# lmcinnes/pynndescent

Hardware: AMD Instinct MI355X
Metric: index build: points indexed/sec (recall@10 vs brute force reported alongside) (higher is better)
Workload: dtype f32

## Files before the change

pynndescent_amd/csrc/sample.hip:

```cpp
#include "common.h"
#include "state.h"

__device__ __forceinline__ uint32_t nnd_offer_salt(uint32_t it_seed, uint32_t u) { return nnd_hash2(it_seed ^ 0x3C6EF372u, u); }

__device__ __forceinline__ uint32_t nnd_offer_slot(uint32_t salt_u, uint32_t v, int rcap) { return nnd_hash2(salt_u ^ 0x68E31DA4u, v) & (uint32_t)(rcap - 1); }
__device__ __forceinline__ int64_t nnd_offer_addr(uint32_t u, uint32_t cls, uint32_t salt_u, uint32_t v, int rcap, int wide) {
    return wide ? (int64_t)u * 2 * rcap + nnd_offer_slot(salt_u, v, 2 * rcap) : ((int64_t)u * 2 + cls) * rcap + nnd_offer_slot(salt_u, v, rcap);
}
__device__ __forceinline__ uint64_t nnd_offer_key(uint32_t slot_word, uint32_t salt_u) {
    return ((uint64_t)slot_word << 32) | (uint64_t)(nnd_unmix32(slot_word) ^ salt_u);
}

__global__ __launch_bounds__(256) void k_sample_reverse(const uint32_t *__restrict__ knn_e, int64_t row_lo, int64_t n, int k, int ks, uint32_t it_seed,
                                                        uint32_t *__restrict__ rbuf, int rcap, int64_t own_lo, int64_t own_hi, int pass,
                                                        uint8_t *__restrict__ active, const int32_t *__restrict__ order, int wide) {
    int64_t b = blockIdx.x;
    if ((gridDim.x & 7) == 0) b = (b & 7) * (gridDim.x >> 3) + (b >> 3);
    const int64_t g = row_lo + b * blockDim.y + threadIdx.y;
    const int j = threadIdx.x;
    if (g >= n || j >= k) return;
    const int64_t v = order ? (int64_t)order[g] : g;
    uint32_t e = knn_e[v * ks + j];
    if (e == NND_EMPTY_E) return;
    uint32_t u = e & NND_IDX_MASK;
    uint32_t cls = e >> 31;
    if (cls != (uint32_t)(pass == 0)) return;
    if (pass == 0 && v >= own_lo && v < own_hi) active[v] = 1;
    if ((int64_t)u < own_lo || (int64_t)u >= own_hi) return;
    if (pass == 0) active[u] = 1;
    else if (!active[u]) return;
    const uint32_t salt = nnd_offer_salt(it_seed, u);
    atomicMin(&rbuf[nnd_offer_addr(u, cls, salt, (uint32_t)v, rcap, wide)], nnd_mix32((uint32_t)v ^ salt));
}

#define SAMPLE_MAX_ITEMS 128

struct sample_scratch {
    uint64_t key[2][SAMPLE_MAX_ITEMS];
};

__global__ __launch_bounds__(256) void k_sample_select(uint32_t *__restrict__ knn_e, int64_t n, int k, int ks, int mc,
                                                       int mcp, uint32_t it_seed, uint32_t *__restrict__ rbuf, int rcap,
                                                       int32_t *__restrict__ cand, int64_t own_lo, int64_t own_hi,
                                                       const uint8_t *__restrict__ active, int wide) {
    __shared__ sample_scratch scr[4];
    const int lane = nnd_lane(), w = threadIdx.x >> 6;
    const int64_t v = own_lo + (int64_t)blockIdx.x * 4 + w;
    if (v >= own_hi) return;
    sample_scratch &sc = scr[w];
    if (!active[v]) {
        for (int j = lane; j < mcp; j += 64) cand[v * 2 * mcp + j] = -1;
        return;
    }

    uint32_t e = NND_EMPTY_E;
    if (lane < k) e = knn_e[v * ks + lane];
    const bool valid = e != NND_EMPTY_E;
    const uint32_t u = e & NND_IDX_MASK;
    const uint32_t cls = e >> 31;
    const uint64_t fkey = ((uint64_t)nnd_hash3(it_seed, (uint32_t)v, u) << 32) | u;
    int cnt[2];
#pragma unroll
    for (int c = 0; c < 2; c++) {
        bool mine = valid && cls == (uint32_t)c;
        unsigned long long m = __ballot(mine);
        if (mine) sc.key[c][nnd_prefix_popc(m)] = fkey;
        cnt[c] = __popcll(m);
    }
    nnd_wave_lds_sync();
    const int nfwd[2] = {cnt[0], cnt[1]};
    const uint32_t salt = nnd_offer_salt(it_seed, (uint32_t)v);
    if (2 * rcap <= 64) {
        const int c = (wide || lane >= rcap) ? 1 : 0;
        uint32_t *slots = rbuf + v * 2 * rcap;
        uint32_t rw = NND_EMPTY_SLOT;
        if (lane < 2 * rcap) {
            rw = slots[lane];
            if (rw != NND_EMPTY_SLOT) slots[lane] = NND_EMPTY_SLOT;
        }
        bool ok = rw != NND_EMPTY_SLOT;
        const uint64_t rk = nnd_offer_key(rw, salt);
        if (ok) {
            const uint32_t src = (uint32_t)rk;
            const int nf = c ? nfwd[1] : nfwd[0];
            for (int j = 0; j < nf; j++) ok &= ((uint32_t)sc.key[c][j] != src);
        }
#pragma unroll
        for (int cc = 0; cc < 2; cc++) {
            const bool mine = ok && c == cc;
            const unsigned long long m = __ballot(mine);
            if (mine) sc.key[cc][cnt[cc] + nnd_prefix_popc(m)] = rk;
            cnt[cc] += __popcll(m);
        }
    } else {
#pragma unroll
        for (int c = 0; c < 2; c++) {
            uint32_t *slots = rbuf + (v * 2 + c) * rcap;
            for (int s0 = 0; s0 < rcap; s0 += 64) {
                int s = s0 + lane;
                uint32_t rw = NND_EMPTY_SLOT;
                if (s < rcap) {
                    rw = slots[s];
                    if (rw != NND_EMPTY_SLOT) slots[s] = NND_EMPTY_SLOT;
                }
                bool ok = rw != NND_EMPTY_SLOT;
                const uint64_t rk = nnd_offer_key(rw, salt);
                if (ok) {
                    uint32_t src = (uint32_t)rk;
                    for (int j = 0; j < nfwd[c]; j++) ok &= ((uint32_t)sc.key[c][j] != src);
                }
                unsigned long long m = __ballot(ok);
                if (ok) sc.key[c][cnt[c] + nnd_prefix_popc(m)] = rk;
                cnt[c] += __popcll(m);
            }
        }
    }
    nnd_wave_lds_sync();

    int32_t *out = cand + v * 2 * mcp;
    int my_rank = 1 << 30;
    const int my_item = (valid && cls == 1u) ? nnd_prefix_popc(__ballot(valid && cls == 1u)) : -1;
#pragma unroll
    for (int c = 0; c < 2; c++) {
        const int M = cnt[c];
        int32_t *dst = out + (c == 1 ? 0 : mcp);
        for (int i0 = 0; i0 < M; i0 += 64) {
            int i = i0 + lane;
            int r = 1 << 30;
            uint64_t key = 0;
            if (i < M) {
                key = sc.key[c][i];
                r = 0;
                for (int j = 0; j < M; j++) r += (sc.key[c][j] < key) ? 1 : 0;
                if (r < mc) dst[r] = (int32_t)(uint32_t)key;
            }
            if (c == 1 && i0 == 0) {
                const int got = __shfl(r, my_item >= 0 ? my_item : 0, 64);
                if (my_item >= 0) my_rank = got;
            }
        }
        int filled = M < mc ? M : mc;
        for (int j = filled + lane; j < mcp; j += 64) dst[j] = -1;
    }
    if (valid && cls == 1u && my_rank < mc) knn_e[v * ks + lane] = u;
}

__global__ __launch_bounds__(256) void k_sample_select_wide(uint32_t *__restrict__ knn_e, int64_t n, int k, int ks, int mc,
                                                            int mcp, uint32_t it_seed, uint32_t *__restrict__ rbuf, int rcap,
                                                            int32_t *__restrict__ cand, int64_t own_lo, int64_t own_hi,
                                                            const uint8_t *__restrict__ active) {
    constexpr int MAXI = NND_WIDE_K + 128;
    __shared__ uint64_t skey[4][2][MAXI];
    __shared__ int srank[4][NND_WIDE_K];
    const int lane = nnd_lane(), w = threadIdx.x >> 6;
    const int64_t v = own_lo + (int64_t)blockIdx.x * 4 + w;
    if (v >= own_hi) return;
    if (!active[v]) {
        for (int j = lane; j < mcp; j += 64) cand[v * 2 * mcp + j] = -1;
        return;
    }
    uint64_t(*key)[MAXI] = skey[w];
    uint32_t e[NND_WIDE_U];
    int item[NND_WIDE_U];
    int cnt[2] = {0, 0};
#pragma unroll
    for (int u = 0; u < NND_WIDE_U; u++) {
        const int j = lane + 64 * u;
        e[u] = j < k ? knn_e[v * ks + j] : NND_EMPTY_E;
        item[u] = -1;
    }
#pragma unroll
    for (int c = 0; c < 2; c++) {
#pragma unroll
        for (int u = 0; u < NND_WIDE_U; u++) {
            const bool mine = e[u] != NND_EMPTY_E && (e[u] >> 31) == (uint32_t)c;
            const unsigned long long m = __ballot(mine);
            if (mine) {
                const uint32_t tgt = e[u] & NND_IDX_MASK;
                item[u] = cnt[c] + nnd_prefix_popc(m);
                key[c][item[u]] = ((uint64_t)nnd_hash3(it_seed, (uint32_t)v, tgt) << 32) | tgt;
            }
            cnt[c] += __popcll(m);
        }
    }
    nnd_wave_lds_sync();
    const int nfwd[2] = {cnt[0], cnt[1]};
    const uint32_t salt = nnd_offer_salt(it_seed, (uint32_t)v);
#pragma unroll
    for (int c = 0; c < 2; c++) {
        uint32_t *slots = rbuf + (v * 2 + c) * rcap;
        for (int s0 = 0; s0 < rcap; s0 += 64) {
            const int sidx = s0 + lane;
            uint32_t rw = NND_EMPTY_SLOT;
            if (sidx < rcap) {
                rw = slots[sidx];
                if (rw != NND_EMPTY_SLOT) slots[sidx] = NND_EMPTY_SLOT;
            }
            bool ok = rw != NND_EMPTY_SLOT;
            const uint64_t rk = nnd_offer_key(rw, salt);
            if (__ballot(ok)) {
                const uint32_t src = (uint32_t)rk;
                for (int j = 0; j < nfwd[c]; j++) ok = ok && ((uint32_t)key[c][j] != src);
            }
            const unsigned long long m = __ballot(ok);
            if (ok) key[c][cnt[c] + nnd_prefix_popc(m)] = rk;
            cnt[c] += __popcll(m);
        }
    }
    nnd_wave_lds_sync();
    int32_t *out = cand + v * 2 * mcp;
#pragma unroll
    for (int c = 0; c < 2; c++) {
        const int M = cnt[c];
        int32_t *dst = out + (c == 1 ? 0 : mcp);
        for (int i0 = 0; i0 < M; i0 += 64) {
            const int i = i0 + lane;
            if (i < M) {
                const uint64_t kk = key[c][i];
                int r = 0;
                for (int j = 0; j < M; j++) r += (key[c][j] < kk) ? 1 : 0;
                if (r < mc) dst[r] = (int32_t)(uint32_t)kk;
                if (c == 1 && i < nfwd[1]) srank[w][i] = r;
            }
        }
        const int filled = M < mc ? M : mc;
        for (int j = filled + lane; j < mcp; j += 64) dst[j] = -1;
    }
    nnd_wave_lds_sync();
#pragma unroll
    for (int u = 0; u < NND_WIDE_U; u++) {
        const int j = lane + 64 * u;
        if (e[u] != NND_EMPTY_E && (e[u] >> 31) == 1u && item[u] >= 0 && srank[w][item[u]] < mc) knn_e[v * ks + j] = e[u] & NND_IDX_MASK;
    }
}

template <bool WIDE>
__device__ __forceinline__ void nnd_select_half(uint32_t *__restrict__ knn_e, int k, int ks, int mc, int mcp, uint32_t it_seed,
                                                int32_t *__restrict__ cand, int64_t vv, bool act, uint32_t e, uint32_t rw0, uint32_t rw1,
                                                uint64_t (*sk)[64], int j, int hb) {
    const uint32_t salt = nnd_offer_salt(it_seed, (uint32_t)vv);
    const uint64_t rk0 = nnd_offer_key(rw0, salt), rk1 = nnd_offer_key(rw1, salt);
    const bool valid = e != NND_EMPTY_E;
    const uint32_t u = e & NND_IDX_MASK;
    const uint32_t cls = e >> 31;
    const uint64_t fkey = ((uint64_t)nnd_hash3(it_seed, (uint32_t)vv, u) << 32) | u;
    const uint32_t below = (1u << j) - 1u;
    int cnt[2];
    uint32_t fmask1 = 0;
#pragma unroll
    for (int c = 0; c < 2; c++) {
        const bool mine = valid && cls == (uint32_t)c;
        const uint32_t hm = (uint32_t)(__ballot(mine) >> hb);
        if (mine) sk[c][__popc(hm & below)] = fkey;
        cnt[c] = __popc(hm);
        if (c == 1) fmask1 = hm;
    }
    nnd_wave_lds_sync();
    const int nf0 = cnt[0], nf1 = cnt[1];
    int32_t *out = cand + vv * 2 * mcp;
    int my_rank = 1 << 30;
    const int my_item = (valid && cls == 1u) ? __popc(fmask1 & below) : -1;
    if constexpr (WIDE) {
        uint64_t *fl = &sk[0][0];
        const uint64_t fk = j < nf1 ? sk[1][j] : NND_EMPTY_KEY;
        nnd_wave_lds_sync();
        if (j < nf1) fl[j] = fk;
        nnd_wave_lds_sync();
        bool ok0 = rw0 != NND_EMPTY_SLOT, ok1 = rw1 != NND_EMPTY_SLOT;
        {
            const int a0 = __builtin_amdgcn_readlane(nf1, 0), a1 = __builtin_amdgcn_readlane(nf1, 32);
            const int nfm = a0 > a1 ? a0 : a1;
            const uint32_t s0 = (uint32_t)rk0, s1 = (uint32_t)rk1;
            for (int q = 0; q < nfm; q++) {
                const uint32_t f = (uint32_t)fl[q];
                ok0 = ok0 && !(q < nf1 && f == s0);
                ok1 = ok1 && !(q < nf1 && f == s1);
            }
        }
        int M = nf1;
        {
            const uint32_t hm0 = (uint32_t)(__ballot(ok0) >> hb), hm1 = (uint32_t)(__ballot(ok1) >> hb);
            if (ok0) fl[M + __popc(hm0 & below)] = rk0;
            M += __popc(hm0);
            if (ok1) fl[M + __popc(hm1 & below)] = rk1;
            M += __popc(hm1);
        }
        nnd_wave_lds_sync();
        const int m0 = __builtin_amdgcn_readlane(M, 0), m1 = __builtin_amdgcn_readlane(M, 32);
        const int mm = m0 > m1 ? m0 : m1;
        const uint64_t key0 = j < M ? fl[j] : NND_EMPTY_KEY, key1 = 32 + j < M ? fl[32 + j] : NND_EMPTY_KEY, key2 = 64 + j < M ? fl[64 + j] : NND_EMPTY_KEY;
        int r0 = 0, r1 = 0, r2 = 0;
        for (int q = 0; q < mm; q++) {
            const uint64_t kq = fl[q];
            const bool in = q < M;
            r0 += (in && kq < key0) ? 1 : 0;
            r1 += (in && kq < key1) ? 1 : 0;
            r2 += (in && kq < key2) ? 1 : 0;
        }
        if (act) {
            if (j < M && r0 < mc) out[r0] = (int32_t)(uint32_t)key0;
            if (32 + j < M && r1 < mc) out[r1] = (int32_t)(uint32_t)key1;
            if (64 + j < M && r2 < mc) out[r2] = (int32_t)(uint32_t)key2;
            const int filled = M < mc ? M : mc;
            for (int q = filled + j; q < mcp; q += 32) out[q] = -1;
            for (int q = j; q < mcp; q += 32) out[mcp + q] = -1;
        }
        const int got = __builtin_amdgcn_ds_bpermute((hb + (my_item >= 0 ? my_item : 0)) << 2, r0);
        if (my_item >= 0) my_rank = got;
        if (act && valid && cls == 1u && my_rank < mc) knn_e[vv * ks + j] = u;
        return;
    }
    bool ok0 = rw0 != NND_EMPTY_SLOT, ok1 = rw1 != NND_EMPTY_SLOT;
    {
        const int a = nf0 > nf1 ? nf0 : nf1;
        const int a0 = __builtin_amdgcn_readlane(a, 0), a1 = __builtin_amdgcn_readlane(a, 32);
        const int nfm = a0 > a1 ? a0 : a1;
        const uint32_t s0 = (uint32_t)rk0, s1 = (uint32_t)rk1;
        for (int q = 0; q < nfm; q++) {
            const uint32_t f0 = (uint32_t)sk[0][q], f1 = (uint32_t)sk[1][q];
            ok0 = ok0 && !(q < nf0 && f0 == s0);
            ok1 = ok1 && !(q < nf1 && f1 == s1);
        }
    }
    {
        const uint32_t hm0 = (uint32_t)(__ballot(ok0) >> hb), hm1 = (uint32_t)(__ballot(ok1) >> hb);
        if (ok0) sk[0][cnt[0] + __popc(hm0 & below)] = rk0;
        if (ok1) sk[1][cnt[1] + __popc(hm1 & below)] = rk1;
        cnt[0] += __popc(hm0);
        cnt[1] += __popc(hm1);
    }
    nnd_wave_lds_sync();

#pragma unroll
    for (int c = 0; c < 2; c++) {
        const int M = cnt[c];
        const int m0 = __builtin_amdgcn_readlane(M, 0), m1 = __builtin_amdgcn_readlane(M, 32);
        const int mm = m0 > m1 ? m0 : m1;
        int32_t *dst = out + (c == 1 ? 0 : mcp);
        const uint64_t key0 = j < M ? sk[c][j] : NND_EMPTY_KEY, key1 = 32 + j < M ? sk[c][32 + j] : NND_EMPTY_KEY;
        int r0 = 0, r1 = 0;
        for (int q = 0; q < mm; q++) {
            const uint64_t kq = sk[c][q];
            const bool in = q < M;
            r0 += (in && kq < key0) ? 1 : 0;
            r1 += (in && kq < key1) ? 1 : 0;
        }
        if (act) {
            if (j < M && r0 < mc) dst[r0] = (int32_t)(uint32_t)key0;
            if (32 + j < M && r1 < mc) dst[r1] = (int32_t)(uint32_t)key1;
            const int filled = M < mc ? M : mc;
            for (int q = filled + j; q < mcp; q += 32) dst[q] = -1;
        }
        if (c == 1) {
            const int got = __builtin_amdgcn_ds_bpermute((hb + (my_item >= 0 ? my_item : 0)) << 2, r0);
            if (my_item >= 0) my_rank = got;
        }
    }
    if (act && valid && cls == 1u && my_rank < mc) knn_e[vv * ks + j] = u;
}

template <int LW>
__device__ __forceinline__ int nnd_group_max(int v) {
    int m = __builtin_amdgcn_readlane(v, 0);
#pragma unroll
    for (int g = LW; g < 64; g += LW) {
        const int o = __builtin_amdgcn_readlane(v, g);
        m = o > m ? o : m;
    }
    return m;
}
template <int LW, int NR>
__device__ __forceinline__ int nnd_select_class(bool act, bool fvalid, uint64_t fkey, const bool (&rvalid)[NR], const uint64_t (&rkey)[NR], int mc,
                                                int mcp, int32_t *dst, uint64_t *list, int j, int gb) {
    constexpr uint32_t GM = LW == 32 ? 0xFFFFFFFFu : ((1u << (LW & 31)) - 1u);
    constexpr int CAP = 2 * LW;
    uint64_t *F = list, *C = list + LW;
    const uint32_t below = (1u << j) - 1u;
    const uint32_t fmask = (uint32_t)(__ballot(fvalid) >> gb) & GM;
    const int nf = __popc(fmask);
    if (fvalid) F[__popc(fmask & below)] = fkey;
    int M = nf;
#pragma unroll
    for (int i = 0; i < NR; i++) M += __popc((uint32_t)(__ballot(rvalid[i]) >> gb) & GM);
    const uint32_t fp = (uint32_t)(fkey >> 32);
    uint32_t rp[NR];
#pragma unroll
    for (int i = 0; i < NR; i++) rp[i] = (uint32_t)(rkey[i] >> 32);
    uint32_t tau = 0xFFFFFFFFu, lo = 0u, hi = 0xFFFFFFFFu;
    if (M > CAP || M > 2 * mc + 4) {
        const float t = (float)(mc + 10) * 4294967296.0f / (float)M;
        tau = t >= 4294967040.0f ? 0xFFFFFFFFu : (uint32_t)t;
    }
    const int nfm = nnd_group_max<LW>(nf);
    int count = 0, cv = 0, tpos = -1, cn = 0;
    uint64_t key0 = NND_EMPTY_KEY, key1 = NND_EMPTY_KEY;
    bool dup0 = false, dup1 = false;
#pragma unroll 1
    for (int iter = 0; iter < 30; iter++) {
        nnd_wave_lds_sync();
        const bool fpass = fvalid && fp <= tau;
        const uint32_t pm = (uint32_t)(__ballot(fpass) >> gb) & GM;
        const int npf = __popc(pm);
        tpos = fpass ? __popc(pm & below) : -1;
        if (fpass) C[tpos] = fkey;
        int pos = npf;
#pragma unroll
        for (int i = 0; i < NR; i++) {
            const bool rpass = rvalid[i] && rp[i] <= tau;
            const uint32_t m = (uint32_t)(__ballot(rpass) >> gb) & GM;
            const int p = pos + __popc(m & below);
            if (rpass && p < CAP) C[p] = rkey[i];
            pos += __popc(m);
        }
        count = pos;
        nnd_wave_lds_sync();
        cn = count < CAP ? count : CAP;
        const bool two = nnd_group_max<LW>(cn) > LW;
        key0 = j < cn ? C[j] : NND_EMPTY_KEY;
        key1 = (two && LW + j < cn) ? C[LW + j] : NND_EMPTY_KEY;
        const bool rev0 = j >= npf && j < cn, rev1 = two && LW + j < cn;
        dup0 = dup1 = false;
        if (__ballot(rev0 || rev1)) {
            const uint32_t s0 = (uint32_t)key0, s1 = (uint32_t)key1;
            if (two) {
#pragma unroll 4
                for (int q = 0; q < nfm; q++) {
                    const uint32_t f = (uint32_t)F[q];
                    dup0 = dup0 || (rev0 && q < nf && f == s0);
                    dup1 = dup1 || (rev1 && q < nf && f == s1);
                }
            } else {
#pragma unroll 4
                for (int q = 0; q < nfm; q++) dup0 = dup0 || (rev0 && q < nf && (uint32_t)F[q] == s0);
            }
        }
        cv = cn - __popc((uint32_t)(__ballot(dup0) >> gb) & GM) - __popc((uint32_t)(__ballot(dup1) >> gb) & GM);
        const bool ok = count <= CAP && (cv >= mc || tau == 0xFFFFFFFFu);
        if (!__ballot(!ok)) break;
        if (!ok) {
            if (count > CAP) {
                hi = tau;
                tau = lo + (hi - lo) / 2;
            } else {
                lo = tau;
                const uint64_t up = (uint64_t)tau + (tau >> 1) + 1u;
                tau = hi == 0xFFFFFFFFu ? (up >= 0xFFFFFFFFull ? 0xFFFFFFFFu : (uint32_t)up) : lo + (hi - lo) / 2 + 1u;
            }
        }
    }
    if (dup0) key0 = NND_EMPTY_KEY;
    if (dup1) key1 = NND_EMPTY_KEY;
    const int cmax = nnd_group_max<LW>(cn);
    nnd_wave_lds_sync();
    C[j] = key0;
    if (cmax > LW) C[LW + j] = key1;
    nnd_wave_lds_sync();
    int r0 = 0, r1 = 0;
    if (cmax > LW) {
#pragma unroll 4
        for (int q = 0; q < cmax; q++) {
            const uint64_t kq = C[q];
            const bool in = q < cn;
            r0 += (in && kq < key0) ? 1 : 0;
            r1 += (in && kq < key1) ? 1 : 0;
        }
    } else {
#pragma unroll 4
        for (int q = 0; q < cmax; q++) r0 += (q < cn && C[q] < key0) ? 1 : 0;
    }
    if (act) {
        if (key0 != NND_EMPTY_KEY && r0 < mc) dst[r0] = (int32_t)(uint32_t)key0;
        if (key1 != NND_EMPTY_KEY && r1 < mc) dst[r1] = (int32_t)(uint32_t)key1;
        const int filled = cv < mc ? cv : mc;
        for (int q = filled + j; q < mcp; q += LW) dst[q] = -1;
    }
    const int got = __builtin_amdgcn_ds_bpermute((gb + (tpos >= 0 ? tpos : 0)) << 2, r0);
    return tpos >= 0 ? got : (1 << 30);
}

template <bool WIDE, int LW, int NRC>
__device__ __forceinline__ void nnd_select_group(uint32_t *__restrict__ knn_e, int k, int ks, int mc, int mcp, uint32_t it_seed,
                                                 int32_t *__restrict__ cand, int64_t vv, bool act, uint32_t e, const uint32_t (&rwo)[NRC],
                                                 const uint32_t (&rwn)[NRC], uint64_t *list, int j, int gb) {
    const uint32_t salt = nnd_offer_salt(it_seed, (uint32_t)vv);
    const bool valid = e != NND_EMPTY_E;
    const uint32_t u = e & NND_IDX_MASK;
    const uint32_t cls = e >> 31;
    const uint64_t fkey = ((uint64_t)nnd_hash3(it_seed, (uint32_t)vv, u) << 32) | u;
    int32_t *out = cand + vv * 2 * mcp;
    int my_rank;
    if constexpr (WIDE) {
        bool rv[2 * NRC];
        uint64_t rk[2 * NRC];
#pragma unroll
        for (int i = 0; i < NRC; i++) {
            rv[i] = rwo[i] != NND_EMPTY_SLOT;
            rk[i] = nnd_offer_key(rwo[i], salt);
            rv[NRC + i] = rwn[i] != NND_EMPTY_SLOT;
            rk[NRC + i] = nnd_offer_key(rwn[i], salt);
        }
        my_rank = nnd_select_class<LW, 2 * NRC>(act, valid, fkey, rv, rk, mc, mcp, out, list, j, gb);
        if (act)
            for (int q = j; q < mcp; q += LW) out[mcp + q] = -1;
    } else {
        bool rv0[NRC], rv1[NRC];
        uint64_t rk0[NRC], rk1[NRC];
#pragma unroll
        for (int i = 0; i < NRC; i++) {
            rv0[i] = rwo[i] != NND_EMPTY_SLOT;
            rk0[i] = nnd_offer_key(rwo[i], salt);
            rv1[i] = rwn[i] != NND_EMPTY_SLOT;
            rk1[i] = nnd_offer_key(rwn[i], salt);
        }
        (void)nnd_select_class<LW, NRC>(act, valid && cls == 0u, fkey, rv0, rk0, mc, mcp, out + mcp, list, j, gb);
        my_rank = nnd_select_class<LW, NRC>(act, valid && cls == 1u, fkey, rv1, rk1, mc, mcp, out, list, j, gb);
    }
    if (act && valid && cls == 1u && my_rank < mc) knn_e[vv * ks + j] = u;
}

template <bool WIDE>
__global__ __launch_bounds__(256) void k_sample_select_h(uint32_t *__restrict__ knn_e, int64_t n, int k, int ks, int mc,
                                                         int mcp, uint32_t it_seed, uint32_t *__restrict__ rbuf,
                                                         int32_t *__restrict__ cand, int64_t own_lo, int64_t own_hi,
                                                         const uint8_t *__restrict__ active) {
    constexpr int RCAP = 32;
    __shared__ uint64_t skey[8][2][64];
    const int lane = nnd_lane(), w = threadIdx.x >> 6, h = lane >> 5, j = lane & 31, hb = lane & 32;
    const int64_t v = own_lo + ((int64_t)blockIdx.x * 4 + w) * 2 + h;
    const bool von = v < own_hi;
    const bool act = von && active[von ? v : own_lo] != 0;
    if (von && !act)
        for (int q = j; q < mcp; q += 32) cand[v * 2 * mcp + q] = -1;
    if (!__ballot(act)) return;
    uint64_t(*sk)[64] = skey[w * 2 + h];
    const int64_t vv = act ? v : own_lo;

    uint32_t e = NND_EMPTY_E;
    if (act && j < k) e = knn_e[vv * ks + j];
    uint32_t rw0 = NND_EMPTY_SLOT, rw1 = NND_EMPTY_SLOT;
    uint32_t *slots = rbuf + vv * 2 * RCAP;
    if (act) {
        rw0 = slots[j];
        rw1 = slots[RCAP + j];
        if (rw0 != NND_EMPTY_SLOT) slots[j] = NND_EMPTY_SLOT;
        if (rw1 != NND_EMPTY_SLOT) slots[RCAP + j] = NND_EMPTY_SLOT;
    }
    nnd_select_half<WIDE>(knn_e, k, ks, mc, mcp, it_seed, cand, vv, act, e, rw0, rw1, sk, j, hb);
}

#define RV_TAB 1024
#ifndef RV_RPT
#define RV_RPT 8
#endif
#define RV_NOHASH 0xFFFFu
#ifndef RV_SEL_THREADS
#define RV_SEL_THREADS 512
#endif

__device__ __forceinline__ uint32_t rv_tab_hash(uint32_t b) { return (b * 2654435761u) >> 22; }

__device__ __forceinline__ int rv_tab_find(volatile uint32_t *hkey, uint32_t b) {
    uint32_t h = rv_tab_hash(b);
#pragma unroll 1
    for (int p = 0; p < 24; p++) {
        uint32_t cur = hkey[h];
        if (cur == 0xFFFFFFFFu) cur = atomicCAS((uint32_t *)&hkey[h], 0xFFFFFFFFu, b);
        if (cur == 0xFFFFFFFFu || cur == b) return (int)h;
        h = (h + 1) & (RV_TAB - 1);
    }
    return -1;
}
#define RV_NOKEY 0xFFFFFFFFu
__device__ __forceinline__ void rv_row_groups(uint32_t key, int &rank, int &size, int &leader) {
    const int lane = (int)__builtin_amdgcn_mbcnt_hi(~0u, __builtin_amdgcn_mbcnt_lo(~0u, 0u));
    rank = 0;
    size = 1;
    leader = lane;
#define RV_ROT(r)                                                                         \
    {                                                                                     \
        const uint32_t ok = (uint32_t)nnd_dpp_i32<NND_DPP_ROW_ROR(r)>((int)key);           \
        const int ol = nnd_dpp_i32<NND_DPP_ROW_ROR(r)>(lane);                              \
        const bool eq = ok == key;                                                        \
        size += eq ? 1 : 0;                                                               \
        rank += (eq && ol < lane) ? 1 : 0;                                                \
        leader = (eq && ol < leader) ? ol : leader;                                       \
    }
    RV_ROT(1) RV_ROT(2) RV_ROT(3) RV_ROT(4) RV_ROT(5) RV_ROT(6) RV_ROT(7) RV_ROT(8)
    RV_ROT(9) RV_ROT(10) RV_ROT(11) RV_ROT(12) RV_ROT(13) RV_ROT(14) RV_ROT(15)
#undef RV_ROT
}
__device__ __forceinline__ uint32_t rv_offer_word(uint32_t it_seed, uint32_t u, uint32_t v) { return nnd_mix32(v ^ nnd_offer_salt(it_seed, u)); }

__global__ __launch_bounds__(256) void k_rev_mark(const uint32_t *__restrict__ knn_e, int64_t row0, int64_t n_rows, int ks, uint8_t *__restrict__ active) {
    const int64_t i = ((int64_t)blockIdx.x * 256 + threadIdx.x) * 4;
    if (i >= n_rows * ks) return;
    const u32x4 e = *(const u32x4 *)(knn_e + row0 * ks + i);
    const int64_t v = row0 + i / ks;
#pragma unroll
    for (int q = 0; q < 4; q++) {
        const uint32_t w = e[q];
        if (w != NND_EMPTY_E && (w >> 31)) {
            active[v] = 1;
            const uint32_t t = w & NND_IDX_MASK;
            if ((uint32_t)(t - (uint32_t)row0) < (uint32_t)n_rows) active[t] = 1;
        }
    }
}
__global__ void k_rev_mark_records(const int32_t *__restrict__ targets, int64_t count, int64_t row0, int64_t n_rows, uint8_t *__restrict__ active) {
    const int64_t i = (int64_t)blockIdx.x * blockDim.x + threadIdx.x;
    if (i >= count) return;
    const uint32_t t = (uint32_t)targets[i];
    const uint32_t u = t & NND_IDX_MASK;
    if ((t >> 31) && (uint32_t)(u - (uint32_t)row0) < (uint32_t)n_rows) active[u] = 1;
}

struct rv_inbox {
    const uint32_t *cursor = nullptr;
    const uint2 *rec = nullptr;
    int cap = 0;
    const uint2 *ov = nullptr;
    const uint32_t *ov_count = nullptr;
};
__global__ __launch_bounds__(256) void k_rev_place(const uint32_t *__restrict__ knn_e, int64_t row0, int64_t n, int k, int ks, uint32_t it_seed,
                                                   const int32_t *__restrict__ order, const int32_t *__restrict__ pos, int logB,
                                                   uint8_t *__restrict__ active, int mark, uint32_t *__restrict__ in_cursor,
                                                   uint2 *__restrict__ in_rec, int cap, uint2 *__restrict__ ov, uint32_t *__restrict__ ov_count) {
    __shared__ uint32_t hkey[RV_TAB], hcnt[RV_TAB], hbase[RV_TAB];
    const int tid = threadIdx.y * blockDim.x + threadIdx.x;
    for (int i = tid; i < RV_TAB; i += 256) { hkey[i] = 0xFFFFFFFFu; hcnt[i] = 0; }
    __syncthreads();
    const int j = threadIdx.x;
    const uint32_t sub = blockIdx.x & 7u, bmask = (1u << logB) - 1u;
    uint32_t ev[RV_RPT], vv[RV_RPT];
#pragma unroll
    for (int it = 0; it < RV_RPT; it++) {
        const int64_t g = ((int64_t)blockIdx.x * RV_RPT + it) * blockDim.y + threadIdx.y;
        ev[it] = NND_EMPTY_E;
        vv[it] = 0;
        if (g < n && j < k) {
            vv[it] = (uint32_t)(order ? order[g] : (int32_t)(row0 + g));
            ev[it] = knn_e[(int64_t)vv[it] * ks + j];
        }
    }
    uint32_t bb[RV_RPT], w[RV_RPT], at[RV_RPT];
    uint16_t m[RV_RPT], hh[RV_RPT];
#pragma unroll
    for (int it = 0; it < RV_RPT; it++) {
        bb[it] = RV_NOKEY;
        w[it] = at[it] = 0;
        m[it] = 0;
        hh[it] = RV_NOHASH;
        if (ev[it] != NND_EMPTY_E && (uint32_t)((ev[it] & NND_IDX_MASK) - (uint32_t)row0) >= (uint32_t)n) {
            if ((ev[it] >> 31) && mark == 1) active[vv[it]] = 1;
            ev[it] = NND_EMPTY_E;
        }
        if (ev[it] != NND_EMPTY_E) {
            const uint32_t u = ev[it] & NND_IDX_MASK, cls = ev[it] >> 31;
            if (cls && mark == 1) { active[vv[it]] = 1; active[u] = 1; }
            if (mark == 2 && !cls && !active[u]) ev[it] = NND_EMPTY_E;
        }
        if (ev[it] != NND_EMPTY_E) {
            const uint32_t u = ev[it] & NND_IDX_MASK, cls = ev[it] >> 31;
            const uint32_t ul = u - (uint32_t)row0;
            const uint32_t p = (uint32_t)(pos ? pos[ul] : (int32_t)ul);
            bb[it] = p >> logB;
            w[it] = rv_offer_word(it_seed, u, vv[it]);
            m[it] = (uint16_t)((p & bmask) | (cls << 15));
        }
    }
#pragma unroll
    for (int it = 0; it < RV_RPT; it++) {
        int rank, size, leader;
        rv_row_groups(bb[it], rank, size, leader);
        int h = -1;
        uint32_t base = 0;
        if (bb[it] != RV_NOKEY && rank == 0) {
            h = rv_tab_find(hkey, bb[it]);
            base = h >= 0 ? atomicAdd(&hcnt[h], (uint32_t)size) : atomicAdd(&in_cursor[(size_t)bb[it] * 8 + sub], (uint32_t)size);
        }
        h = __shfl(h, leader, 64);
        base = (uint32_t)__shfl((int)base, leader, 64);
        if (bb[it] != RV_NOKEY) {
            hh[it] = h >= 0 ? (uint16_t)h : RV_NOHASH;
            at[it] = base + (uint32_t)rank;
        }
    }
    __syncthreads();
    for (int i = tid; i < RV_TAB; i += 256)
        if (hcnt[i]) hbase[i] = atomicAdd(&in_cursor[(size_t)hkey[i] * 8 + sub], hcnt[i]);
    __syncthreads();
#pragma unroll
    for (int it = 0; it < RV_RPT; it++) {
        if (bb[it] == RV_NOKEY) continue;
        const uint32_t at_ = hh[it] == RV_NOHASH ? at[it] : hbase[hh[it]] + at[it];
        if (at_ < (uint32_t)cap)
            in_rec[((size_t)bb[it] * 8 + sub) * cap + at_] = make_uint2(w[it], (uint32_t)m[it]);
        else
            ov[atomicAdd(ov_count, 1u)] = make_uint2(w[it], (bb[it] << 9) | (((uint32_t)m[it] >> 15) << 8) | ((uint32_t)m[it] & 0xFFu));
    }
}
__global__ __launch_bounds__(256) void k_rev_import(const int32_t *__restrict__ targets, const uint32_t *__restrict__ sources, int64_t count,
                                                    uint32_t it_seed, int64_t row0, int64_t n, const int32_t *__restrict__ pos, int logB,
                                                    const uint8_t *__restrict__ active, int filter, uint32_t *__restrict__ in_cursor,
                                                    uint2 *__restrict__ in_rec, int cap, uint2 *__restrict__ ov, uint32_t *__restrict__ ov_count) {
    const int64_t i = (int64_t)blockIdx.x * 256 + threadIdx.x;
    if (i >= count) return;
    const uint32_t t = (uint32_t)targets[i];
    const uint32_t cls = t >> 31, u = t & NND_IDX_MASK, ul = u - (uint32_t)row0;
    if (ul >= (uint32_t)n || (filter && !cls && !active[u])) return;
    const uint32_t p = (uint32_t)(pos ? pos[ul] : (int32_t)ul);
    const uint32_t b = p >> logB, tl = p & ((1u << logB) - 1u);
    const uint32_t w = rv_offer_word(it_seed, u, sources[i]);
    const size_t sr = (size_t)b * 8 + (threadIdx.x & 7);
    const uint32_t at = atomicAdd(&in_cursor[sr], 1u);
    if (at < (uint32_t)cap) {
        in_rec[sr * cap + at] = make_uint2(w, tl | (cls << 15));
    } else {
        ov[atomicAdd(ov_count, 1u)] = make_uint2(w, (b << 9) | (cls << 8) | tl);
    }
}
template <typename F>
__device__ __forceinline__ void rv_each_record(const rv_inbox &ib, int64_t b, int tid, int nthr, F f) {
    uint32_t c[8], pre[9];
    bool over = false;
#pragma unroll
    for (int sr = 0; sr < 8; sr++) c[sr] = ib.cursor[b * 8 + sr];
    pre[0] = 0;
#pragma unroll
    for (int sr = 0; sr < 8; sr++) {
        over = over || c[sr] > (uint32_t)ib.cap;
        pre[sr + 1] = pre[sr] + (c[sr] < (uint32_t)ib.cap ? c[sr] : (uint32_t)ib.cap);
    }
    const uint2 *base = ib.rec + (size_t)b * 8 * ib.cap;
    for (uint32_t i = tid; i < pre[8]; i += nthr) {
        int sr = 0;
#pragma unroll
        for (int q = 1; q < 8; q++) sr += i >= pre[q] ? 1 : 0;
        uint32_t lo = pre[0];
#pragma unroll
        for (int q = 1; q < 8; q++) lo = sr >= q ? pre[q] : lo;
        const uint2 r = base[(size_t)sr * ib.cap + (i - lo)];
        f(r.x, r.y);
    }
    if (over) {
        const uint32_t M = *ib.ov_count;
        for (uint32_t i = tid; i < M; i += nthr) {
            const uint2 r = ib.ov[i];
            if ((int64_t)(r.y >> 9) == b) f(r.x, (r.y & 0xFFu) | (((r.y >> 8) & 1u) << 15));
        }
    }
}

__device__ __forceinline__ uint32_t rv_ovf_slot(uint32_t word, uint32_t cap) { return nnd_mix32(word ^ 0x68E31DA4u) & (cap - 1u); }

template <int RCAP, int NB, bool WIDE>
__global__ __launch_bounds__(1024) void k_rev_fill(rv_inbox ib, int64_t row0, int64_t n, const int32_t *__restrict__ order,
                                                   const uint8_t *__restrict__ active, uint32_t *__restrict__ rbuf) {
    constexpr int ROW = 2 * RCAP;
    constexpr int CAP = WIDE ? 2 * RCAP : RCAP;
    constexpr int NBANK = WIDE ? NB : 2 * NB;
    __shared__ uint32_t bank[NB * ROW];
    __shared__ uint32_t cnt[NBANK];
    __shared__ int any_ovf;
    const int tid = threadIdx.x;
    const int64_t b = blockIdx.x;
    for (int i = tid; i < NB * ROW; i += 1024) bank[i] = NND_EMPTY_SLOT;
    for (int i = tid; i < NBANK; i += 1024) cnt[i] = 0;
    if (tid == 0) any_ovf = 0;
    __syncthreads();
    rv_each_record(ib, b, tid, 1024, [&](uint32_t w, uint32_t m) {
        const uint32_t bk = WIDE ? (m & 0x7FFFu) : ((m & 0x7FFFu) * 2 + (m >> 15));
        const uint32_t s = atomicAdd(&cnt[bk], 1u);
        if (s < (uint32_t)CAP) bank[bk * CAP + s] = w;
    });
    __syncthreads();
    for (int i = tid; i < NBANK; i += 1024)
        if (cnt[i] > (uint32_t)CAP) any_ovf = 1;
    __syncthreads();
    if (any_ovf) {
        for (int i = tid; i < NBANK * CAP; i += 1024)
            if (cnt[i / CAP] > (uint32_t)CAP) bank[i] = NND_EMPTY_SLOT;
        __syncthreads();
        rv_each_record(ib, b, tid, 1024, [&](uint32_t w, uint32_t m) {
            const uint32_t bk = WIDE ? (m & 0x7FFFu) : ((m & 0x7FFFu) * 2 + (m >> 15));
            if (cnt[bk] > (uint32_t)CAP) atomicMin(&bank[bk * CAP + rv_ovf_slot(w, CAP)], w);
        });
        __syncthreads();
    }
    const int tl0 = tid / ROW, c = tid % ROW;
    for (int tl = tl0; tl < NB; tl += 1024 / ROW) {
        const int64_t p = b * NB + tl;
        if (p >= n) break;
        const int64_t v = order ? (int64_t)order[p] : row0 + p;
        if (!active[v]) continue;
        rbuf[v * ROW + c] = bank[tl * ROW + c];
    }
}

template <bool WIDE, int LW>
__global__ __launch_bounds__(RV_SEL_THREADS) void k_rev_select(rv_inbox ib, int64_t row0, int64_t n, const int32_t *__restrict__ order,
                                                    const uint8_t *__restrict__ active,
                                                    uint32_t *__restrict__ knn_e, int k, int ks, int mc, int mcp, uint32_t it_seed,
                                                    int32_t *__restrict__ cand) {
    constexpr int RCAP = 32, NB = 128, ROW = 2 * RCAP, NT = RV_SEL_THREADS, NG = NT / LW, PER = NB / NG, NRC = RCAP / LW;
    constexpr int CAP = WIDE ? 2 * RCAP : RCAP;
    constexpr int NBANK = WIDE ? NB : 2 * NB;
    __shared__ uint32_t bank[NB * ROW];
    __shared__ uint32_t cnt[NBANK];
    __shared__ uint64_t skey[NG][LW == 32 ? 128 : 3 * LW];
    __shared__ int32_t vtx[NB];
    __shared__ int any_ovf;
    const int tid = threadIdx.x, lane = tid & 63, grp = tid / LW, j = lane & (LW - 1), gb = lane & (64 - LW);
    const int64_t b = blockIdx.x;
    if (tid < NB) {
        const int64_t p = b * NB + tid;
        int32_t v = -1;
        if (p < n) {
            v = order ? order[p] : (int32_t)(row0 + p);
            if (!active[v]) v = -2 - v;
        }
        vtx[tid] = v;
    }
    for (int i = tid; i < NB * ROW; i += NT) bank[i] = NND_EMPTY_SLOT;
    for (int i = tid; i < NBANK; i += NT) cnt[i] = 0;
    if (tid == 0) any_ovf = 0;
    __syncthreads();
    uint32_t pre_e = NND_EMPTY_E;
    {
        const int32_t v0 = vtx[grp];
        if (v0 >= 0 && j < k) pre_e = knn_e[(int64_t)v0 * ks + j];
    }
    rv_each_record(ib, b, tid, NT, [&](uint32_t w, uint32_t m) {
        const uint32_t bk = WIDE ? (m & 0x7FFFu) : ((m & 0x7FFFu) * 2 + (m >> 15));
        const uint32_t sl = atomicAdd(&cnt[bk], 1u);
        if (sl < (uint32_t)CAP) bank[bk * CAP + sl] = w;
    });
    __syncthreads();
    for (int i = tid; i < NBANK; i += NT)
        if (cnt[i] > (uint32_t)CAP) any_ovf = 1;
    __syncthreads();
    if (any_ovf) {
        for (int i = tid; i < NBANK * CAP; i += NT)
            if (cnt[i / CAP] > (uint32_t)CAP) bank[i] = NND_EMPTY_SLOT;
        __syncthreads();
        rv_each_record(ib, b, tid, NT, [&](uint32_t w, uint32_t m) {
            const uint32_t bk = WIDE ? (m & 0x7FFFu) : ((m & 0x7FFFu) * 2 + (m >> 15));
            if (cnt[bk] > (uint32_t)CAP) atomicMin(&bank[bk * CAP + rv_ovf_slot(w, CAP)], w);
        });
        __syncthreads();
    }
    uint64_t *sk = skey[grp];
#pragma unroll 1
    for (int r = 0; r < PER; r++) {
        const int tl = r * NG + grp;
        const int32_t v = vtx[tl];
        const bool act = v >= 0;
        const uint32_t e = pre_e;
        pre_e = NND_EMPTY_E;
        if (r + 1 < PER) {
            const int32_t vn = vtx[tl + NG];
            if (vn >= 0 && j < k) pre_e = knn_e[(int64_t)vn * ks + j];
        }
        if (v <= -2)
            for (int q = j; q < mcp; q += LW) cand[(int64_t)(-2 - v) * 2 * mcp + q] = -1;
        if (!__ballot(act)) continue;
        uint32_t rwo[NRC], rwn[NRC];
#pragma unroll
        for (int i = 0; i < NRC; i++) {
            rwo[i] = act ? bank[tl * ROW + i * LW + j] : NND_EMPTY_SLOT;
            rwn[i] = act ? bank[tl * ROW + RCAP + i * LW + j] : NND_EMPTY_SLOT;
        }
        nnd_wave_lds_sync();
#ifdef NND_RV_NOSELECT
        if (e == 0x12345u && rwo[0] == 7u && rwn[0] == 9u) cand[0] = 1;
        continue;
#endif
        if constexpr (LW == 32)
            nnd_select_half<WIDE>(knn_e, k, ks, mc, mcp, it_seed, cand, act ? (int64_t)v : 0, act, e, rwo[0], rwn[0], (uint64_t(*)[64])sk, j, gb);
        else
            nnd_select_group<WIDE, LW, NRC>(knn_e, k, ks, mc, mcp, it_seed, cand, act ? (int64_t)v : 0, act, e, rwo, rwn, sk, j, gb);
    }
}

__global__ void k_rev_invert(const int32_t *__restrict__ order, int64_t row0, int64_t n, int32_t *__restrict__ pos) {
    const int64_t g = (int64_t)blockIdx.x * blockDim.x + threadIdx.x;
    if (g < n) pos[order[g] - row0] = (int32_t)g;
}

static bool sample_wide(const nnd_ctx *ctx) { return ctx->all_new && ctx->rcap == 32 && ctx->k <= 64; }

static void launch_reverse_pass(nnd_ctx *ctx, int pass, uint32_t it_seed) {
    const bool shard = ctx->n_ranks > 1;
    const int64_t row_lo = shard ? ctx->own_lo : 0, row_hi = shard ? ctx->own_hi : ctx->n;
    int ksp = 16;
    while (ksp < ctx->ks) ksp <<= 1;
    const int rows = 256 / ksp;
    unsigned grid = (unsigned)((row_hi - row_lo + rows - 1) / rows);
    grid = (grid + 7u) & ~7u;
    const int32_t *order = (!shard && ctx->forest_built && ctx->p.n_trees > 0) ? ctx->perm[ctx->cur] : nullptr;
    ctx->rbuf_clean = false;
    hipLaunchKernelGGL(k_sample_reverse, dim3(grid), dim3(ksp, rows), 0, ctx->stream, ctx->knn_e, row_lo, row_hi, ctx->k, ctx->ks,
                       it_seed, ctx->rbuf, ctx->rcap, ctx->own_lo, ctx->own_hi, pass, ctx->active, order, sample_wide(ctx) ? 1 : 0);
}

static uint32_t sample_seed(const nnd_ctx *ctx) { return nnd_hash2(ctx->seed ^ 0x9E3779B9u, (uint32_t)ctx->iter + 1u); }

static void launch_select(nnd_ctx *ctx, uint32_t it_seed, bool wide) {
    if (ctx->k > 64 || ctx->mc > 64) {
        hipLaunchKernelGGL(k_sample_select_wide, dim3((unsigned)((ctx->own_hi - ctx->own_lo + 3) / 4)), dim3(256), 0, ctx->stream,
                           ctx->knn_e, ctx->n, ctx->k, ctx->ks, ctx->mc, ctx->mcp, it_seed, ctx->rbuf, ctx->rcap, ctx->cand, ctx->own_lo,
                           ctx->own_hi, ctx->active);
        if (ctx->n_ranks <= 1) ctx->rbuf_clean = true;
        return;
    }
    const bool force_old = (ctx->p.flags & NND_FLAG_TEST_SELECT_WAVE) != 0;
    if (ctx->k <= 32 && ctx->rcap == 32 && ctx->mc <= 32 && !force_old) {
        auto kern = wide ? k_sample_select_h<true> : k_sample_select_h<false>;
        hipLaunchKernelGGL(kern, dim3((unsigned)((ctx->own_hi - ctx->own_lo + 7) / 8)), dim3(256), 0, ctx->stream,
                           ctx->knn_e, ctx->n, ctx->k, ctx->ks, ctx->mc, ctx->mcp, it_seed, ctx->rbuf, ctx->cand, ctx->own_lo,
                           ctx->own_hi, ctx->active);
        if (ctx->n_ranks <= 1) ctx->rbuf_clean = true;
        return;
    }
    hipLaunchKernelGGL(k_sample_select, dim3((unsigned)((ctx->own_hi - ctx->own_lo + 3) / 4)), dim3(256), 0, ctx->stream,
                       ctx->knn_e, ctx->n, ctx->k, ctx->ks, ctx->mc, ctx->mcp, it_seed, ctx->rbuf, ctx->rcap, ctx->cand, ctx->own_lo,
                       ctx->own_hi, ctx->active, wide ? 1 : 0);
    if (ctx->n_ranks <= 1) ctx->rbuf_clean = true;
}

static int rv_prepare(nnd_ctx *ctx, int logB, const int32_t *order, int64_t row0, int64_t n_rows, int64_t extra, int *cap_out) {
    const int64_t nb = ((n_rows - 1) >> logB) + 1, nov = n_rows * ctx->k + extra;
    const int64_t mean = n_rows * ctx->k / (nb * 8) + 1;
    int64_t cap64 = (ctx->k <= 32 ? 4 : 2) * mean;
    cap64 = cap64 < 64 ? 64 : ((cap64 + 63) / 64) * 64;
    const int cap = (int)cap64;
    *cap_out = cap;
    const int64_t need = nb * 8 * cap;
    bool ok = !(ctx->p.flags & NND_FLAG_TEST_SAMPLE_NOMEM);
    if (ok) {
        if (cap != ctx->rv_in_cap) ctx->rv_cap_in = 0;
        ok = ctx->mem.grow2(&ctx->rv_in_cursor, (size_t)nb * 8 + 8, &ctx->rv_in_rec, (size_t)need, &ctx->rv_cap_in, need, need);
        if (ok) ctx->rv_in_cap = cap;
    }
    ok = ok && ctx->mem.grow(&ctx->rv_ov, &ctx->rv_cap_ov, nov, extra > 0 ? nov + nov / 4 : nov);
    if (ok && order && (!ctx->rv_pos || ctx->rv_pos_gen != ctx->forest_gen || ctx->rv_pos_of != order)) {
        ok = ctx->mem.grow(&ctx->rv_pos, &ctx->rv_cap_pos, n_rows, n_rows);
        if (ok) {
            hipLaunchKernelGGL(k_rev_invert, dim3((unsigned)((n_rows + 255) / 256)), dim3(256), 0, ctx->stream, order, row0, n_rows, ctx->rv_pos);
            ctx->rv_pos_gen = ctx->forest_gen;
            ctx->rv_pos_of = order;
        }
    }
    if (!ok) {
        ctx->mem.free(&ctx->rv_in_cursor);
        ctx->mem.free(&ctx->rv_in_rec);
        ctx->mem.free(&ctx->rv_ov);
        ctx->rv_cap_in = ctx->rv_cap_ov = 0;
        ctx->rv_in_cap = 0;
        ctx->rv_off = true;
        NND_HIP_CHECK(hipMemsetAsync(ctx->rbuf + (size_t)ctx->slim_row0() * 2 * ctx->rcap, 0xFF, sizeof(uint32_t) * (size_t)ctx->slim_rows() * 2 * ctx->rcap, ctx->stream));
        ctx->rbuf_clean = true;
        return 2;
    }
    return 0;
}

static bool rv_fused(const nnd_ctx *ctx) {
    return ctx->k <= 32 && ctx->rcap == 32 && ctx->mc <= 32 && !(ctx->p.flags & NND_FLAG_TEST_SELECT_WAVE);
}
static bool rv_bucketed(const nnd_ctx *ctx) { return (ctx->rcap == 32 || ctx->rcap == 64) && !ctx->rv_off && !(ctx->p.flags & NND_FLAG_TEST_SAMPLE_ATOMIC); }
static int launch_sample_bucketed(nnd_ctx *ctx, uint32_t it_seed, bool wide, const int32_t *in_targets, const uint32_t *in_sources, int64_t n_in) {
    const bool fused = rv_fused(ctx), shard = ctx->n_ranks > 1;
    const int logB = (fused || ctx->rcap != 32) ? 7 : 8;
    const int64_t row0 = shard ? ctx->own_lo : 0, n_rows = shard ? ctx->own_hi - ctx->own_lo : ctx->n;
    if (n_rows <= 0) return 0;
    const int32_t *order = shard ? ctx->own_order : ((ctx->forest_built && ctx->p.n_trees > 0) ? ctx->perm[ctx->cur] : nullptr);
    int cap = 0;
    if (const int prc = rv_prepare(ctx, logB, order, row0, n_rows, n_in, &cap)) return prc;
    const int32_t *pos = order ? ctx->rv_pos : nullptr;
    const int64_t nb = ((n_rows - 1) >> logB) + 1;
    if (nb >= ((int64_t)1 << 23)) { ctx->set_error("candidate sampling: %lld buckets exceed the 2^23 bucket ids of an overflow record", (long long)nb); return 1; }
    int ksp = 16;
    while (ksp < ctx->ks) ksp <<= 1;
    const int rows = 256 / ksp;
    const unsigned grid = (unsigned)((n_rows + (int64_t)rows * RV_RPT - 1) / ((int64_t)rows * RV_RPT));
    hipStream_t st = ctx->stream;
    uint32_t *ov_count = ctx->rv_in_cursor + (size_t)nb * 8;
    NND_HIP_CHECK(hipMemsetAsync(ctx->rv_in_cursor, 0, sizeof(uint32_t) * ((size_t)nb * 8 + 8), st));
    NND_HIP_CHECK(hipMemsetAsync(ctx->active + row0, ctx->all_new ? 1 : 0, (size_t)n_rows, st));
    int mark = ctx->all_new ? 0 : 1;
    if (mark == 1 && (shard || (ctx->last_updates >= 0 && ctx->last_updates * 8 < ctx->n * ctx->k))) {
        hipLaunchKernelGGL(k_rev_mark, dim3((unsigned)((n_rows * ctx->ks / 4 + 255) / 256)), dim3(256), 0, st, ctx->knn_e, row0, n_rows, ctx->ks, ctx->active);
        if (n_in > 0)
            hipLaunchKernelGGL(k_rev_mark_records, dim3((unsigned)((n_in + 255) / 256)), dim3(256), 0, st, in_targets, n_in, row0, n_rows, ctx->active);
        mark = 2;
    }
    hipLaunchKernelGGL(k_rev_place, dim3(grid), dim3(ksp, rows), 0, st, ctx->knn_e, row0, n_rows, ctx->k, ctx->ks, it_seed, order, pos, logB, ctx->active,
                       mark, ctx->rv_in_cursor, ctx->rv_in_rec, cap, ctx->rv_ov, ov_count);
    if (n_in > 0)
        hipLaunchKernelGGL(k_rev_import, dim3((unsigned)((n_in + 255) / 256)), dim3(256), 0, st, in_targets, in_sources, n_in, it_seed, row0, n_rows, pos, logB,
                           ctx->active, mark == 2 ? 1 : 0, ctx->rv_in_cursor, ctx->rv_in_rec, cap, ctx->rv_ov, ov_count);
    rv_inbox ib;
    ib.cursor = ctx->rv_in_cursor;
    ib.rec = ctx->rv_in_rec;
    ib.cap = cap;
    ib.ov = ctx->rv_ov;
    ib.ov_count = ov_count;
    if (fused) {
        const bool q16 = ctx->ks == 16 && ctx->mc <= 16 && !(ctx->p.flags & NND_FLAG_TEST_SELECT_HALF);
        auto kern = q16 ? (wide ? k_rev_select<true, 16> : k_rev_select<false, 16>) : (wide ? k_rev_select<true, 32> : k_rev_select<false, 32>);
        hipLaunchKernelGGL(kern, dim3((unsigned)nb), dim3(RV_SEL_THREADS), 0, st, ib, row0, n_rows, order, ctx->active, ctx->knn_e, ctx->k, ctx->ks, ctx->mc, ctx->mcp,
                           it_seed, ctx->cand);
        return 0;
    }
    ctx->rbuf_clean = false;
    auto fill = ctx->rcap == 32 ? (wide ? k_rev_fill<32, 256, true> : k_rev_fill<32, 256, false>) : k_rev_fill<64, 128, false>;
    hipLaunchKernelGGL(fill, dim3((unsigned)nb), dim3(1024), 0, st, ib, row0, n_rows, order, ctx->active, ctx->rbuf);
    launch_select(ctx, it_seed, wide);
    return 0;
}

int nnd_launch_sample(nnd_ctx *ctx) {
    if (ctx->n_ranks > 1) {
        ctx->set_error("nnd_launch_sample: this handle is one shard of a row-sharded build; use nnd_sample_begin / nnd_sample_finish");
        return 1;
    }
    const uint32_t it_seed = sample_seed(ctx);
    if (rv_bucketed(ctx)) {
        const bool wide_b = sample_wide(ctx);
        const int brc = launch_sample_bucketed(ctx, it_seed, wide_b, nullptr, nullptr, 0);
        if (brc == 1) return 1;
        if (brc == 0) {
            ctx->all_new = false;
            NND_HIP_CHECK(hipGetLastError());
            return 0;
        }
    }
    NND_HIP_CHECK(hipMemsetAsync(ctx->active, 0, (size_t)ctx->n, ctx->stream));
    const int n_pass = ctx->all_new ? 1 : 2;
    const bool wide = sample_wide(ctx);
    for (int pass = 0; pass < n_pass; pass++) launch_reverse_pass(ctx, pass, it_seed);
    ctx->all_new = false;
    launch_select(ctx, it_seed, wide);
    NND_HIP_CHECK(hipGetLastError());
    return 0;
}

#define OFFER_IT 16
__global__ __launch_bounds__(256) void k_offer_export(const uint32_t *__restrict__ knn_e, int64_t row_lo, int64_t row_hi, int k, int ks,
                                                      uint32_t it_seed, const int64_t *__restrict__ bounds, int n_ranks,
                                                      int64_t own_lo, int64_t own_hi, int64_t cap, long long *__restrict__ cursors,
                                                      int32_t *__restrict__ targets, uint32_t *__restrict__ sources,
                                                      long long *__restrict__ dropped) {
    __shared__ int cnt[64];
    __shared__ long long base[64];
    const int tid = threadIdx.y * blockDim.x + threadIdx.x;
    if (tid < 64) cnt[tid] = 0;
    __syncthreads();
    const int j = threadIdx.x;
    uint32_t ev[OFFER_IT];
    int dest[OFFER_IT], my[OFFER_IT];
#pragma unroll
    for (int it = 0; it < OFFER_IT; it++) {
        const int64_t g = row_lo + ((int64_t)blockIdx.x * OFFER_IT + it) * blockDim.y + threadIdx.y;
        ev[it] = NND_EMPTY_E;
        if (g < row_hi && j < k) ev[it] = knn_e[g * ks + j];
    }
#pragma unroll
    for (int it = 0; it < OFFER_IT; it++) {
        dest[it] = -1;
        my[it] = 0;
        if (ev[it] != NND_EMPTY_E) {
            const int64_t u = (int64_t)(ev[it] & NND_IDX_MASK);
            if (u < own_lo || u >= own_hi) dest[it] = nnd_owner_of(bounds, n_ranks, u);
        }
        unsigned long long todo = __ballot(dest[it] >= 0);
        while (todo) {
            const int lead = __builtin_ctzll(todo);
            const int dd = __builtin_amdgcn_readlane(dest[it], lead);
            const unsigned long long md = __ballot(dest[it] == dd);
            int b = 0;
            if ((tid & 63) == lead) b = atomicAdd(&cnt[dd], __popcll(md));
            b = __builtin_amdgcn_readlane(b, lead);
            if (dest[it] == dd) my[it] = b + nnd_prefix_popc(md);
            todo &= ~md;
        }
    }
    __syncthreads();
    if (tid < n_ranks && cnt[tid] > 0) base[tid] = (long long)atomicAdd((unsigned long long *)&cursors[tid], (unsigned long long)cnt[tid]);
    __syncthreads();
    int n_drop = 0;
#pragma unroll
    for (int it = 0; it < OFFER_IT; it++) {
        if (dest[it] < 0) continue;
        const int64_t g = row_lo + ((int64_t)blockIdx.x * OFFER_IT + it) * blockDim.y + threadIdx.y;
        const uint32_t u = ev[it] & NND_IDX_MASK, cls = ev[it] >> 31;
        const long long at = base[dest[it]] + my[it];
        if (at < cap) {
            const int64_t idx = (int64_t)dest[it] * cap + at;
            targets[idx] = (int32_t)(u | (cls << 31));
            sources[idx] = (uint32_t)g;
        } else {
            n_drop++;
        }
    }
    if (n_drop) atomicAdd((unsigned long long *)dropped, (unsigned long long)n_drop);
}

__global__ void k_offer_import(const int32_t *__restrict__ targets, const uint32_t *__restrict__ sources, int64_t count, uint32_t want_cls,
                               uint32_t it_seed, uint32_t *__restrict__ rbuf, int rcap, uint8_t *__restrict__ active,
                               int64_t own_lo, int64_t own_hi, int wide) {
    const int64_t i = (int64_t)blockIdx.x * blockDim.x + threadIdx.x;
    if (i >= count) return;
    const uint32_t t = (uint32_t)targets[i];
    const uint32_t cls = t >> 31, u = t & NND_IDX_MASK;
    if (cls != want_cls || (int64_t)u < own_lo || (int64_t)u >= own_hi) return;
    if (cls == 1u) active[u] = 1;
    else if (!active[u]) return;
    const uint32_t v = sources[i];
    const uint32_t salt = nnd_offer_salt(it_seed, u);
    atomicMin(&rbuf[nnd_offer_addr(u, cls, salt, v, rcap, wide)], nnd_mix32(v ^ salt));
}

int nnd_launch_sample_begin(nnd_ctx *ctx, int64_t cap, int32_t *targets_dev, uint32_t *sources_dev, long long *counts_dev) {
    if (ctx->n_ranks < 1 || !ctx->shard_bounds) { ctx->set_error("nnd_sample_begin: call nnd_set_shard_bounds first"); return 1; }
    const uint32_t it_seed = sample_seed(ctx);
    NND_HIP_CHECK(hipMemsetAsync(ctx->shard_cursors, 0, sizeof(long long) * 66, ctx->stream));
    if (!rv_bucketed(ctx)) {
        NND_HIP_CHECK(hipMemsetAsync(ctx->active + ctx->slim_row0(), 0, (size_t)ctx->slim_rows(), ctx->stream));
        launch_reverse_pass(ctx, 0, it_seed);
    }
    if (ctx->n_ranks > 1) {
        int ksp = 16;
        while (ksp < ctx->ks) ksp <<= 1;
        const int rows = 256 / ksp;
        const unsigned grid = (unsigned)((ctx->own_hi - ctx->own_lo + (int64_t)rows * OFFER_IT - 1) / ((int64_t)rows * OFFER_IT));
        if (grid > 0)
            hipLaunchKernelGGL(k_offer_export, dim3(grid), dim3(ksp, rows), 0, ctx->stream, ctx->knn_e, ctx->own_lo, ctx->own_hi, ctx->k,
                               ctx->ks, it_seed, ctx->shard_bounds, ctx->n_ranks, ctx->own_lo, ctx->own_hi, cap, ctx->shard_cursors,
                               targets_dev, sources_dev, ctx->shard_cursors + 64);
    }
    NND_HIP_CHECK(hipGetLastError());
    NND_HIP_CHECK(hipMemcpyAsync(counts_dev, ctx->shard_cursors, sizeof(long long) * (size_t)ctx->n_ranks, hipMemcpyDeviceToDevice, ctx->stream));
    return 0;
}

int nnd_launch_sample_finish(nnd_ctx *ctx, const int32_t *targets_dev, const uint32_t *sources_dev, int64_t count) {
    const uint32_t it_seed = sample_seed(ctx);
    const unsigned grid = (unsigned)((count + 255) / 256);
    const bool wide = sample_wide(ctx);
    if (rv_bucketed(ctx)) {
        const int brc = launch_sample_bucketed(ctx, it_seed, wide, targets_dev, sources_dev, count);
        if (brc == 1) return 1;
        if (brc == 0) {
            ctx->all_new = false;
            NND_HIP_CHECK(hipGetLastError());
            return 0;
        }
        NND_HIP_CHECK(hipMemsetAsync(ctx->active + ctx->slim_row0(), 0, (size_t)ctx->slim_rows(), ctx->stream));
        launch_reverse_pass(ctx, 0, it_seed);
    }
    if (count > 0) {
        ctx->rbuf_clean = false;
        hipLaunchKernelGGL(k_offer_import, dim3(grid), dim3(256), 0, ctx->stream, targets_dev, sources_dev, count, 1u, it_seed, ctx->rbuf,
                           ctx->rcap, ctx->active, ctx->own_lo, ctx->own_hi, wide ? 1 : 0);
    }
    if (!ctx->all_new) {
        launch_reverse_pass(ctx, 1, it_seed);
        if (count > 0)
            hipLaunchKernelGGL(k_offer_import, dim3(grid), dim3(256), 0, ctx->stream, targets_dev, sources_dev, count, 0u, it_seed, ctx->rbuf,
                               ctx->rcap, ctx->active, ctx->own_lo, ctx->own_hi, 0);
    }
    ctx->all_new = false;
    launch_select(ctx, it_seed, wide);
    NND_HIP_CHECK(hipGetLastError());
    return 0;
}
```

Baseline: 52.28 million.

## Compact active vertices in rev_select and skip empty blocks

Builds a compacted list of active and inactive vertices per block using wave ballots and popcounts. The select loop then iterates only over active vertices instead of all slots, and inactive vertices get their candidate rows cleared in a separate cooperative loop. Blocks with no active vertices exit early without initializing the bank or reading the inbox. This removes wasted select rounds and LDS setup when many vertices are inactive in later iterations, at the cost of extra ballots, a second barrier and an index indirection.

Result: no change. 52.62 million (median of 6 runs) (+0.7%).

```diff
diff --git a/pynndescent_amd/csrc/sample.hip b/pynndescent_amd/csrc/sample.hip
--- a/pynndescent_amd/csrc/sample.hip
+++ b/pynndescent_amd/csrc/sample.hip
@@ -802,34 +802,58 @@
                                                     const uint8_t *__restrict__ active,
                                                     uint32_t *__restrict__ knn_e, int k, int ks, int mc, int mcp, uint32_t it_seed,
                                                     int32_t *__restrict__ cand) {
-    constexpr int RCAP = 32, NB = 128, ROW = 2 * RCAP, NT = RV_SEL_THREADS, NG = NT / LW, PER = NB / NG, NRC = RCAP / LW;
+    constexpr int RCAP = 32, NB = 128, ROW = 2 * RCAP, NT = RV_SEL_THREADS, NG = NT / LW, NRC = RCAP / LW;
     constexpr int CAP = WIDE ? 2 * RCAP : RCAP;
     constexpr int NBANK = WIDE ? NB : 2 * NB;
     __shared__ uint32_t bank[NB * ROW];
     __shared__ uint32_t cnt[NBANK];
     __shared__ uint64_t skey[NG][LW == 32 ? 128 : 3 * LW];
     __shared__ int32_t vtx[NB];
+    __shared__ uint8_t lst[NB];
+    __shared__ int wn[2][2];
     __shared__ int any_ovf;
     const int tid = threadIdx.x, lane = tid & 63, grp = tid / LW, j = lane & (LW - 1), gb = lane & (64 - LW);
     const int64_t b = blockIdx.x;
+    int32_t v_own = -1;
+    uint64_t am = 0, im = 0;
     if (tid < NB) {
         const int64_t p = b * NB + tid;
-        int32_t v = -1;
         if (p < n) {
-            v = order ? order[p] : (int32_t)(row0 + p);
-            if (!active[v]) v = -2 - v;
-        }
-        vtx[tid] = v;
-    }
-    for (int i = tid; i < NB * ROW; i += NT) bank[i] = NND_EMPTY_SLOT;
-    for (int i = tid; i < NBANK; i += NT) cnt[i] = 0;
-    if (tid == 0) any_ovf = 0;
-    __syncthreads();
+            v_own = order ? order[p] : (int32_t)(row0 + p);
+            if (!active[v_own]) v_own = -2 - v_own;
+        }
+        vtx[tid] = v_own;
+        am = __ballot(v_own >= 0);
+        im = __ballot(v_own <= -2);
+        if (lane == 0) {
+            wn[tid >> 6][0] = __popcll(am);
+            wn[tid >> 6][1] = __popcll(im);
+        }
+    }
+    auto arm = [&]() {
+        for (int i = tid; i < NB * ROW; i += NT) bank[i] = NND_EMPTY_SLOT;
+        for (int i = tid; i < NBANK; i += NT) cnt[i] = 0;
+        if (tid == 0) any_ovf = 0;
+    };
+    if constexpr (WIDE) arm();
+    __syncthreads();
+    const int n_act = wn[0][0] + wn[1][0], n_off = wn[0][1] + wn[1][1];
+    if (tid < NB) {
+        const uint64_t below = (1ull << lane) - 1ull;
+        const int w = tid >> 6;
+        if (v_own >= 0) lst[(w ? wn[0][0] : 0) + __popcll(am & below)] = (uint8_t)tid;
+        else if (v_own <= -2) lst[NB - 1 - ((w ? wn[0][1] : 0) + __popcll(im & below))] = (uint8_t)tid;
+    }
+    if constexpr (!WIDE)
+        if (n_act) arm();
+    __syncthreads();
+    for (int a = tid >> 4; a < n_off; a += NT / 16) {
+        const int64_t vi = -2 - vtx[lst[NB - 1 - a]];
+        for (int q = tid & 15; q < mcp; q += 16) cand[vi * 2 * mcp + q] = -1;
+    }
+    if (n_act == 0) return;
     uint32_t pre_e = NND_EMPTY_E;
-    {
-        const int32_t v0 = vtx[grp];
-        if (v0 >= 0 && j < k) pre_e = knn_e[(int64_t)v0 * ks + j];
-    }
+    if (grp < n_act && j < k) pre_e = knn_e[(int64_t)vtx[lst[grp]] * ks + j];
     rv_each_record(ib, b, tid, NT, [&](uint32_t w, uint32_t m) {
         const uint32_t bk = WIDE ? (m & 0x7FFFu) : ((m & 0x7FFFu) * 2 + (m >> 15));
         const uint32_t sl = atomicAdd(&cnt[bk], 1u);
@@ -850,19 +874,16 @@
         __syncthreads();
     }
     uint64_t *sk = skey[grp];
+    const int rounds = (n_act + NG - 1) / NG;
 #pragma unroll 1
-    for (int r = 0; r < PER; r++) {
-        const int tl = r * NG + grp;
-        const int32_t v = vtx[tl];
-        const bool act = v >= 0;
+    for (int r = 0; r < rounds; r++) {
+        const int a = r * NG + grp;
+        const bool act = a < n_act;
+        const int tl = act ? (int)lst[a] : 0;
+        const int32_t v = act ? vtx[tl] : 0;
         const uint32_t e = pre_e;
         pre_e = NND_EMPTY_E;
-        if (r + 1 < PER) {
-            const int32_t vn = vtx[tl + NG];
-            if (vn >= 0 && j < k) pre_e = knn_e[(int64_t)vn * ks + j];
-        }
-        if (v <= -2)
-            for (int q = j; q < mcp; q += LW) cand[(int64_t)(-2 - v) * 2 * mcp + q] = -1;
+        if (a + NG < n_act && j < k) pre_e = knn_e[(int64_t)vtx[lst[a + NG]] * ks + j];
         if (!__ballot(act)) continue;
         uint32_t rwo[NRC], rwn[NRC];
 #pragma unroll
@@ -876,9 +897,9 @@
         continue;
 #endif
         if constexpr (LW == 32)
-            nnd_select_half<WIDE>(knn_e, k, ks, mc, mcp, it_seed, cand, act ? (int64_t)v : 0, act, e, rwo[0], rwn[0], (uint64_t(*)[64])sk, j, gb);
+            nnd_select_half<WIDE>(knn_e, k, ks, mc, mcp, it_seed, cand, (int64_t)v, act, e, rwo[0], rwn[0], (uint64_t(*)[64])sk, j, gb);
         else
-            nnd_select_group<WIDE, LW, NRC>(knn_e, k, ks, mc, mcp, it_seed, cand, act ? (int64_t)v : 0, act, e, rwo, rwn, sk, j, gb);
+            nnd_select_group<WIDE, LW, NRC>(knn_e, k, ks, mc, mcp, it_seed, cand, (int64_t)v, act, e, rwo, rwn, sk, j, gb);
     }
 }
 
```
